# PolusAI/nyxus

Measured on AMD Instinct MI355X. Metric: ROIs/sec (*ALL_GLCM*+*ALL_INTENSITY*, 1024^2 tiles), higher is better.
Workload: dtype f64; 1 GPU; *ALL_GLCM*+*ALL_INTENSITY*, coarse_gray_depth=8, 4 angles, d=1, 1000 synthetic 1024x1024 tiles/GPU x 196 ROIs/tile (disk r=30, 2821 px, bbox 61x61), intensities U[1,4095]; reduce stage on pre-assembled ROI clouds resident in HBM; n_columns=185

## Files before the change

nyxus_amd/csrc/roi_features.hip:

```cpp
#include <hip/hip_runtime.h>
#include <type_traits>
#include <algorithm>
#include <cstdio>
#include "knobs.h"
#include "device_math.h"
#include "roi_kernel.h"
#include "launch_util.h"
#include "glcm_rows.h"
#include "glcm_w64.h"
#include "intensity_close.h"
#include "sort_lds.h"
#include "../../include/nyxhip.h"

namespace nyxhip {


enum { S_MEAN = 0, S_P10, S_P90, S_MEDIAN, S_MODE, S_NG };


template <int NW> __device__ __forceinline__ double xw_chain(const double* s_red, int k)
{
    return NW == 1 ? s_red[k] : ((s_red[k] + s_red[8 + k]) + s_red[16 + k]) + s_red[24 + k];
}
template <int NW> __device__ __forceinline__ double xw_pairs(const double* s_red, int k)
// ... 442 lines not shown
        f[G_DIFAVE] = davg;
        f[G_DIFVAR] = dv;
        f[G_IDMN] = sm[8 + 6];
        f[G_ID] = sm[8 + 7];
        f[G_IDN] = sm[8 + 8];
        f[G_IV] = sm[8 + 9];
        const double r1 = (ent_t - hxy1_t) / hx;
        f[G_INFOMEAS1] = isfinite(r1) ? r1 : soft_nan;
        if (empty)
            for (int k = 0; k < kGlcmAngled; k++) f[k] = soft_nan;
    }
    wav_sync<false>();
}

typedef unsigned short us2_t __attribute__((ext_vector_type(2)));
#ifdef NYX_G16_EXIT
#define G16_EXIT(k, keep) do { if ((k) == NYX_G16_EXIT) { ((double*)blk)[lane & 31] = (double)(keep); return; } } while (0)
#else
#define G16_EXIT(k, keep) do { } while (0)
#endif
template <int NG, int ROLE = 0>
__device__ __forceinline__ void glcm_features_wave64_v2(const uint16_t* P, int Ng_rt, uint32_t* blk, double soft_nan, int lane)
{
    const int Ng = NG ? NG : Ng_rt;
    typedef __attribute__((address_space(3))) const uint16_t lds_cu16_t;
    typedef __attribute__((address_space(3))) const uint32_t lds_cu32_t;
    typedef __attribute__((address_space(3))) uint32_t lds_u32_t;
    const int pitch = (Ng + 3) & ~1;
    double* const f = (double*)blk;
    double* const sm = f + 32;
    double* const T2 = f + 64;
    const bool act = lane < Ng;
    const uint16_t* const Pd = P + pitch;
    G16_EXIT(0, lane);
    uint32_t rc = 0;
    {
        const int nw = (Ng + 1) >> 1;
        lds_cu32_t* rw = (lds_cu32_t*)(uintptr_t)(Pd + (act ? lane : 0) * pitch);
        us2_t a2 = {0, 0};
#pragma unroll 8
        for (int j = 0; j < nw; j++) a2 = a2 + __builtin_bit_cast(us2_t, rw[j]);
        rc = act ? (uint32_t)a2.x + (uint32_t)a2.y : 0u;
    }
    G16_EXIT(1, rc);
    if constexpr (ROLE == 2) {
        const int cj = lane < Ng ? lane : Ng;
        lds_cu16_t* pc = (lds_cu16_t*)(uintptr_t)(Pd + cj);
        uint32_t cc2 = 0;
#pragma unroll 8
        for (int i = 0; i < Ng; i++) cc2 += pc[i * pitch];
        if (!act) cc2 = 0;
        const uint32_t csum2 = wave_sum_t<uint32_t>(rc);
        const double sum_p2 = csum2 == 0 ? 1.0 : (double)csum2;
        const double pcol = fdiv((double)cc2, sum_p2), prow = fdiv((double)rc, sum_p2);
        double hxy1c = 0, hxy2 = 0;
        unsigned long long rem = __ballot(act && rc != 0u);
        while (rem) {
            const int r0 = (int)__builtin_ctzll(rem);
            const uint32_t v = (uint32_t)__builtin_amdgcn_readlane((int)rc, r0);
            const unsigned long long pbits = (unsigned long long)__double_as_longlong(prow);
            const double pr = __longlong_as_double((long long)(((unsigned long long)(uint32_t)__builtin_amdgcn_readlane((int)(uint32_t)(pbits >> 32), r0) << 32) |
                                                               (uint32_t)__builtin_amdgcn_readlane((int)(uint32_t)pbits, r0)));
            unsigned long long grp = __ballot(act && rc == v);
            rem &= ~grp;
            const double pp = pcol * pr;
            const double lg = (double)fast_log2f(pp + 0.000000001);
            hxy2 = __builtin_fma(pp * (double)(uint32_t)__popcll(grp), lg, hxy2);
            uint32_t gsum = 0;
            while (grp) {
                const int r = (int)__builtin_ctzll(grp);
                grp &= grp - 1ull;
                gsum += pc[r * pitch];
            }
            hxy1c = __builtin_fma((double)gsum, lg, hxy1c);
        }
        blk_sync<false>();
        T2[lane] = hxy1c;
        f[lane] = hxy2;
        blk_sync<false>();
        return;
    }
    uint32_t cc = 0, dc = 0;
    uint32_t pxpy_c[2] = {0u, 0u};
    {
        uint32_t W = 0, X = 0;
        const int cj = lane < Ng ? lane : Ng;
        lds_cu16_t* pc = (lds_cu16_t*)(uintptr_t)(Pd + cj);
        lds_u32_t* const b0 = (lds_u32_t*)(uintptr_t)blk;
        lds_u32_t* px = lane == 0 ? b0 : b0 + 128 + lane;
        lds_u32_t* pw = lane == Ng - 1 ? b0 + 64 : b0 + 128 + lane;
#pragma unroll 8
        for (int i = 0; i < Ng; i++) {
            const uint32_t cnt = pc[i * pitch];
            cc += cnt;
            X = lane_plus1_z(X) + cnt;
            W = lane_minus1_z(W) + cnt;
            px[i] = X;
            pw[i] = W;
        }
        wav_sync<false>();
        const uint32_t dlo = act ? blk[lane] : 0u;
        const uint32_t eup = act ? blk[64 + Ng - 1 - lane] : 0u;
        wav_sync<false>();
        const uint32_t wrev = (uint32_t)__builtin_amdgcn_ds_bpermute(4 * (Ng - 1 - lane), (int)W);
        dc = act ? eup + (lane >= 1 ? wrev : 0u) : 0u;
        const int k1 = lane + 64;
        const uint32_t xa = (uint32_t)__builtin_amdgcn_ds_bpermute(4 * (lane - (Ng - 1)), (int)X);
        const uint32_t xb = (uint32_t)__builtin_amdgcn_ds_bpermute(4 * (k1 - (Ng - 1)), (int)X);
        pxpy_c[0] = lane < Ng ? dlo : (lane <= 2 * Ng - 2 ? xa : 0u);
        pxpy_c[1] = k1 <= 2 * Ng - 2 ? xb : 0u;
        if (!act) cc = 0;
    }
    G16_EXIT(2, rc + cc + dc + pxpy_c[0] + pxpy_c[1]);
    const uint32_t csum = wave_sum_t<uint32_t>(rc);
    const bool empty = csum == 0;
    const double sum_p = empty ? 1.0 : (double)csum;
    const double inv_sum_p = fdiv(1.0, sum_p);
    const double pcol = fdiv((double)cc, sum_p), prow = fdiv((double)rc, sum_p), pxmy = fdiv((double)dc, sum_p);
    double pxpy[2] = {0.0, 0.0};
#pragma unroll
    for (int u = 0; u < 2; u++)
        if (lane + 64 * u < 2 * Ng - 1) pxpy[u] = fdiv((double)pxpy_c[u], sum_p);

    {
        const int ca = lane & 7;
        const double pk = (double)ca * inv_sum_p;
        const double t = ca < 7 ? pk * (double)fast_log2f(pk + 0.000000001) : 0.0;
        if (lane < 8) sm[lane] = t;
        wav_sync<false>();
        T2[lane] = t + sm[lane >> 3];
        wav_sync<false>();
    }
    G16_EXIT(3, (uint32_t)(pcol + prow + pxmy + pxpy[0] + pxpy[1]));
    double ent = 0;
    uint32_t asm_i = 0, cmax = 0;
    {
        const int half = (Ng + 1) >> 1, l32 = lane & 31;
        const bool hi = lane >= 32, colp = 2 * l32 < Ng;
        lds_cu32_t* pwd = (lds_cu32_t*)(uintptr_t)(Pd + (hi ? half : 0) * pitch) + (colp ? l32 : 0);
        typedef __attribute__((address_space(3))) const double lds_cd_t;
        lds_cd_t* const T2l = (lds_cd_t*)(uintptr_t)T2;
        us2_t mx = {0, 0};
#pragma unroll 8
        for (int s = 0; s < half; s++) {
            uint32_t w = pwd[s * (pitch >> 1)];
            if (Ng & 1) w = (colp && (!hi || s + half < Ng)) ? w : 0u;
            else if (Ng < 64) w = colp ? w : 0u;
            const us2_t v = __builtin_bit_cast(us2_t, w);
            asm_i = __builtin_amdgcn_udot2(v, v, asm_i, false);
            mx = __builtin_elementwise_max(mx, v);
            const uint32_t m = __builtin_bit_cast(uint32_t, __builtin_elementwise_min(v, (us2_t){7, 7}));
            ent += T2l[(m & 7u) | (m >> 13)];
        }
        cmax = mx.x > mx.y ? (uint32_t)mx.x : (uint32_t)mx.y;
    }
    G16_EXIT(4, (uint32_t)(pcol + prow + pxmy + pxpy[0] + pxpy[1] + ent) + asm_i + cmax);
    double hxy1c = 0, hxy2 = 0;
    if constexpr (ROLE == 0) {
        const int cj = lane < Ng ? lane : Ng;
        lds_cu16_t* pc = (lds_cu16_t*)(uintptr_t)(Pd + cj);
        unsigned long long rem = __ballot(act && rc != 0u);
        while (rem) {
            const int r0 = (int)__builtin_ctzll(rem);
            const uint32_t v = (uint32_t)__builtin_amdgcn_readlane((int)rc, r0);
            const unsigned long long pbits = (unsigned long long)__double_as_longlong(prow);
            const double pr = __longlong_as_double((long long)(((unsigned long long)(uint32_t)__builtin_amdgcn_readlane((int)(uint32_t)(pbits >> 32), r0) << 32) |
                                                               (uint32_t)__builtin_amdgcn_readlane((int)(uint32_t)pbits, r0)));
            unsigned long long grp = __ballot(act && rc == v);
            rem &= ~grp;
            const double pp = pcol * pr;
            const double lg = (double)fast_log2f(pp + 0.000000001);
            hxy2 = __builtin_fma(pp * (double)(uint32_t)__popcll(grp), lg, hxy2);
            uint32_t gsum = 0;
            while (grp) {
                const int r = (int)__builtin_ctzll(grp);
                grp &= grp - 1ull;
                gsum += pc[r * pitch];
            }
            hxy1c = __builtin_fma((double)gsum, lg, hxy1c);
        }
    }
    if (__ballot(cmax >= 7u)) {
        const int cj = lane < Ng ? lane : Ng;
        lds_cu16_t* pc = (lds_cu16_t*)(uintptr_t)(Pd + cj);
        unsigned long long rem = __ballot(act && rc != 0u);
        while (rem) {
            const int r = (int)__builtin_ctzll(rem);
            rem &= rem - 1ull;
            const uint32_t cnt = pc[r * pitch];
            if (cnt >= 7u) { const double p = (double)cnt * inv_sum_p; ent += p * (double)fast_log2f(p + 0.000000001); }
        }
    }
    if constexpr (ROLE == 1) {
        blk_sync<false>();
        blk_sync<false>();
        hxy1c = T2[lane];
        hxy2 = f[lane];
        wav_sync<false>();
    }
    G16_EXIT(5, (uint32_t)(pcol + prow + pxmy + pxpy[0] + pxpy[1] + ent + hxy1c + hxy2) + asm_i + cmax);
    glcm_w64_tail<NG>(Ng, lane, rc, cc, dc, pxpy_c, csum, sum_p, inv_sum_p, pcol, prow, pxmy, pxpy, ent, hxy1c, hxy2, asm_i, cmax, f);
}

#ifdef NYX_STAMP
#define STAMP(i)                                                                          \
    do {                                                                                  \
        unsigned long long t__ = __builtin_readcyclecounter();                            \
        if (tid == 0 && A.stamps) atomicAdd(&A.stamps[i], t__ - t_prev__);                \
        t_prev__ = __builtin_readcyclecounter();                                          \
    } while (0)
#elif defined(NYX_EXIT_AT)
#define STAMP(i) do { if ((i) == NYX_EXIT_AT) return; } while (0)
#else
#define STAMP(i) do { } while (0)
#endif

__constant__ const double kPctFrac[8] = {0.01, 0.1, 0.25, 0.75, 0.9, 0.99, 0.5, 0.5};

typedef __attribute__((address_space(3))) uint8_t lds_u8_t;

typedef const __attribute__((address_space(4))) RoiArgs KArgs;
__device__ __forceinline__ KArgs* late_kernarg()
{
    KArgs* p = (KArgs*)__builtin_amdgcn_kernarg_segment_ptr();
    asm volatile("" : "+s"(p));
    return p;
}
template <bool LATE>
struct KView {
    const RoiArgs& a;
    KArgs* p;
    __device__ __forceinline__ explicit KView(const RoiArgs& a_) : a(a_), p(LATE ? late_kernarg() : nullptr) {}
    __device__ __forceinline__ auto operator->() const
    {
        if constexpr (LATE) return p;
        else return &a;
    }
};
template <bool GS, bool C16, bool SPLIT, bool D8, int FAM = 0, int TIER = 4, bool G16 = false, int WIN = 2, int NW = 4, bool DEFER_P = false>
__device__ __forceinline__ void roi_features_body(const RoiArgs& A, const uint64_t slot)
{
    static_assert((NW == 4 && NW == kMaxAngles) || (NW == 8 && G16 && FAM == 4), "one workgroup of four waves per ROI (and a wave per GLCM angle)");
    constexpr int BS = NW * 64;
    extern __shared__ __attribute__((aligned(16))) unsigned char lds_raw[];
    unsigned char* const lds = GS ? A.sp.scratch + (size_t)blockIdx.x * A.sp.stride : lds_raw;
    const int tid = (int)threadIdx.x, lane = tid & 63, wave = __builtin_amdgcn_readfirstlane(tid >> 6);
    uint64_t roi;
    if (!roi_of_slot(A.sp, slot, A.n_roi, roi))
        return;

    auto reg = [&](uint32_t o) -> unsigned char* { return (GS && o < A.L.gs_lds_bytes) ? lds_raw + o : lds + o; };
    double* s_red = (double*)reg(A.L.red);
    double* s_stat = (double*)reg(A.L.stat);
    uint32_t* s_lbc = (uint32_t*)reg(A.L.lbc);
    uint32_t* s_val = (uint32_t*)(lds + A.L.val);
    using dense_t = typename std::conditional<D8, uint8_t, uint16_t>::type;
    dense_t* s_dense = (dense_t*)(lds + (D8 ? 0u : A.L.dense));
    uint16_t* s_lvlmap = (uint16_t*)reg(A.L.lvlmap);
    uint32_t* s_P = (uint32_t*)reg(A.L.P);
    double* s_g = (double*)reg(A.L.gscr);

    const uint64_t off = A.px_offset[roi];
    const uint32_t n = (uint32_t)(A.px_offset[roi + 1] - off);
    const uint32_t w = A.bbox_w[roi], h = A.bbox_h[roi];
    const uint32_t area = w * h;
    const uint32_t vmin = A.min_inten[roi], vmax = A.max_inten[roi];
    if (!roi_in_launch(A.sp, n, w, h, vmax - vmin))
        return;
    if (vmax - vmin < A.sp.min_range || (A.sp.max_range != 0u && vmax - vmin > A.sp.max_range))
        return;
    constexpr bool FAST = FAM == 1 || FAM == 3;
    constexpr int kRowsTag = 16 + TIER * 4 + (C16 ? 2 : 0) + (D8 ? 1 : 0);
    const bool do_int = FAM == 1 || FAM == 2 || (FAM == 0 && (A.mask & NYXHIP_FAM_INTENSITY) != 0);
    const bool do_glcm = FAM == 1 || FAM == 3 || FAM == 4 || (FAM == 0 && (A.mask & NYXHIP_FAM_GLCM) != 0);
    double* const out_row = A.out + roi * A.ld;
#ifdef NYX_STAMP
    unsigned long long t_prev__ = __builtin_readcyclecounter();
#endif

    const uint32_t range = vmax - vmin;
    const bool use_count = C16 ? do_int : (do_int && A.L.count_cap != 0 && range < A.L.count_cap);
    if (C16 && do_int && range >= A.L.count_cap) {
        if (tid == 0) atomicCAS(A.status, 0, NYXHIP_ERR_ROI_TOO_LARGE);
        return;
    }
    uint32_t* s_cnt = (uint32_t*)reg(A.L.cnt);
    uint32_t P2 = 1;
    while (P2 < n)
        P2 <<= 1;
    const bool radix = !C16 && A.L.radix != 0;
    const bool k16 = radix && A.L.radix_k16 != 0;
    if (n == 0 || (do_int && ((use_count || radix) ? n : P2) > A.L.sort_cap) || (do_glcm && area > A.L.dense_cap)) {
        if (SPLIT && A.glcm_ng && tid == 0)
            A.glcm_ng[roi] = 0;
        if (n != 0 && A.sp.defer_large)
            return;
        if (tid == 0 && n != 0)
            atomicCAS(A.status, 0, NYXHIP_ERR_ROI_TOO_LARGE);
        for (int c = tid; c < A.n_cols; c += BS)
            out_row[c] = __longlong_as_double(0x7ff8000000000000LL);
        return;
    }

    const int greyInfo = A.ibsi ? 0 : A.grey_depth;
    if (FAST) __builtin_assume(greyInfo > 0 && greyInfo <= 16);
    if (G16) __builtin_assume(greyInfo > 16 && greyInfo <= 64);
    const double mslope = greyInfo > 0 ? (double)greyInfo / ((double)vmax - 0.) : 0.0;

    for (int c = tid; c < A.n_cols; c += BS)
        out_row[c] = 0.0;
    if (do_glcm) {
        uint32_t* d32 = (uint32_t*)s_dense;
        for (uint32_t i = tid; i < (D8 ? (area + 64 + 3) / 4 : (area + 1) / 2); i += BS)
            d32[i] = 0;
        if (greyInfo < 0)
            for (uint32_t i = tid; i <= A.L.lvl_cap; i += BS)
                s_lvlmap[i] = 0;
    }
    if (do_int) {
        if (use_count) {
            uint4* c4 = (uint4*)s_cnt;
            const uint32_t n16 = C16 ? (range + 8) / 8 : (range + 4) / 4;
            for (uint32_t i = tid; i < n16; i += BS)
                c4[i] = make_uint4(0, 0, 0, 0);
        } else if (!radix) {
            for (uint32_t i = n + tid; i < P2; i += BS)
                s_val[i] = 0xFFFFFFFFu;
        }
    }
    if (tid < 16)
        s_stat[tid] = 0.0;
    grp_sync<GS, NW>();

    STAMP(0);
    unsigned long long sum = 0, sumsq = 0;
    uint32_t lvl_max = 0;
    constexpr int kU = 4;
    const bool small_v = vmax < (1u << 24);
    const __amdgpu_buffer_rsrc_t rs_v = __builtin_amdgcn_make_buffer_rsrc((void*)(A.inten + off), 0, (int)(n * 4u), 0x00020000);
    const __amdgpu_buffer_rsrc_t rs_x = __builtin_amdgcn_make_buffer_rsrc((void*)(A.x + off), 0, (int)(n * 2u), 0x00020000);
    const __amdgpu_buffer_rsrc_t rs_y = __builtin_amdgcn_make_buffer_rsrc((void*)(A.y + off), 0, (int)(n * 2u), 0x00020000);
    auto trip = [&](auto full_c, auto nz_c, auto tiny_c, uint32_t base) {
        constexpr bool FULL = decltype(full_c)::value, NZ = decltype(nz_c)::value, TINY = decltype(tiny_c)::value;
        uint32_t v[kU], px[kU], py[kU];
#pragma unroll
        for (int u = 0; u < kU; u++) {
            const uint32_t i = base + u * BS + tid;
            v[u] = __builtin_amdgcn_raw_buffer_load_b32(rs_v, (int)(i * 4u), 0, 0);
            px[u] = do_glcm ? (uint32_t)(uint16_t)__builtin_amdgcn_raw_buffer_load_b16(rs_x, (int)(i * 2u), 0, 0) : 0u;
            py[u] = do_glcm ? (uint32_t)(uint16_t)__builtin_amdgcn_raw_buffer_load_b16(rs_y, (int)(i * 2u), 0, 0) : 0u;
        }
        uint32_t s32 = 0, q32 = 0;
        const uint32_t i0 = base + tid;
        uint16_t* const val16 = (uint16_t*)s_val + i0;
#pragma unroll
        for (int u = 0; u < kU; u++) {
            if (!FULL && i0 + u * BS >= n)
                continue;
            if (do_int) {
                if (C16) val16[u * BS] = (uint16_t)(v[u] - vmin);
                else if (k16) ((uint16_t*)s_val)[i0 + u * BS] = (uint16_t)(v[u] - vmin);
                else s_val[i0 + u * BS] = v[u];
                const uint32_t sq = (TINY || small_v) ? (uint32_t)__umul24(v[u], v[u]) : (uint32_t)(v[u] * v[u]);
                if (TINY) { s32 += v[u]; q32 += sq; }
                else { sum += v[u]; sumsq += sq; }
                if (use_count)
                {
                    const uint32_t ci = v[u] - vmin;
                    if (C16) atomicAdd(cnt16_word(s_cnt, ci), 1u << (16 * (ci & 1u)));
                    else atomicAdd(&s_cnt[ci], 1u);
                }
            }
            if (do_glcm) {
                uint32_t lvl = 0;
                if (NZ || v[u] != 0) {
                    if (FAST || G16) {
                        const uint32_t sc = (uint32_t)(mslope * (double)v[u] + 1.0);
                        lvl = sc > (uint32_t)greyInfo ? (uint32_t)greyInfo : sc;
                    } else
                    lvl = greyInfo > 0 ? bin_matlab(v[u], mslope, greyInfo)
                        : greyInfo < 0 ? bin_radiomix(v[u], vmin, vmax, -greyInfo) : v[u];
                    if (greyInfo < 0)
                        s_lvlmap[lvl] = 1;
                    if (greyInfo <= 0)
                        lvl_max = lvl > lvl_max ? lvl : lvl_max;
                }
                const uint32_t cell = __umul24(py[u], w) + px[u];
                if (D8)
                    *(lds_u8_t*)(cell < area ? cell : area + 64) = (uint8_t)lvl;
                else if (cell < area)
                    s_dense[cell] = (dense_t)(lvl > 0xFFFFu ? 0xFFFFu : lvl);
            }
        }
        if (TINY) { sum += s32; sumsq += q32; }
    };
    bool from_window = false;
    if constexpr (WIN != 0 && !GS) {
    if (WIN == 1 || A.win.inten != nullptr) {
        from_window = true;
        const uint32_t L = A.win.label[roi], x0 = A.win.x0[roi];
        const uint64_t tile_px = (uint64_t)A.win.H * A.win.W;
        const bool nz_w = vmin > 0;
        auto member = [&](uint32_t v, uint32_t i, uint32_t cell) {
            if (do_int) {
                if (C16 || k16) ((uint16_t*)s_val)[i] = (uint16_t)(v - vmin);
                else s_val[i] = v;
                sum += v;
                sumsq += small_v ? mul24(v, v) : (uint32_t)(v * v);
                if (use_count) {
                    const uint32_t ci = v - vmin;
                    if (C16) atomicAdd(cnt16_word(s_cnt, ci), 1u << (16 * (ci & 1u)));
                    else atomicAdd(&s_cnt[ci], 1u);
                }
            }
            if (do_glcm) {
                uint32_t lvl = 0;
                if (nz_w || v != 0) {
                    if (FAST || G16) {
                        const uint32_t sc = (uint32_t)(mslope * (double)v + 1.0);
                        lvl = sc > (uint32_t)greyInfo ? (uint32_t)greyInfo : sc;
                    } else
                    lvl = greyInfo > 0 ? bin_matlab(v, mslope, greyInfo) : greyInfo < 0 ? bin_radiomix(v, vmin, vmax, -greyInfo) : v;
                    if (greyInfo < 0) s_lvlmap[lvl] = 1;
                    if (greyInfo <= 0) lvl_max = lvl > lvl_max ? lvl : lvl_max;
                }
                if (D8) *(lds_u8_t*)cell = (uint8_t)lvl;
                else s_dense[cell] = (dense_t)(lvl > 0xFFFFu ? 0xFFFFu : lvl);
            }
        };
        if (w <= 64 && tile_px * 4ull < (1ull << 31)) {
            constexpr int UW = 4;
            const int dtl = A.win.dt_label, dti = A.win.dt_inten;
            auto window_load = [&](auto DTL_c, auto DTI_c) {
            constexpr int DTLc = decltype(DTL_c)::value, DTIc = decltype(DTI_c)::value;
            const int dtl = DTLc ? DTLc : A.win.dt_label, dti = DTIc ? DTIc : A.win.dt_inten;
            const uint32_t Wt = A.win.W;
            const uint64_t tile0 = (uint64_t)A.win.tile[roi] * tile_px;
            const __amdgpu_buffer_rsrc_t rs_l = __builtin_amdgcn_make_buffer_rsrc((void*)((const char*)A.win.lab + tile0 * (uint64_t)dtl), 0, (int)(tile_px * (uint64_t)dtl), 0x00020000);
            const __amdgpu_buffer_rsrc_t rs_i = __builtin_amdgcn_make_buffer_rsrc((void*)((const char*)A.win.inten + tile0 * (uint64_t)dti), 0, (int)(tile_px * (uint64_t)dti), 0x00020000);
            auto ldb = [](const __amdgpu_buffer_rsrc_t& rs, uint32_t voff, uint32_t soff, int dt) -> uint32_t {
                return dt == 4 ? (uint32_t)__builtin_amdgcn_raw_buffer_load_b32(rs, (int)voff, (int)soff, 0)
                     : dt == 2 ? (uint32_t)(uint16_t)__builtin_amdgcn_raw_buffer_load_b16(rs, (int)voff, (int)soff, 0)
                               : (uint32_t)(uint8_t)__builtin_amdgcn_raw_buffer_load_b8(rs, (int)voff, (int)soff, 0);
            };
            const uint32_t e0 = (A.win.y0[roi] + (uint32_t)wave) * Wt + x0;
            const uint32_t vl = (uint32_t)lane * (uint32_t)dtl, vi = (uint32_t)lane * (uint32_t)dti;
            const bool incol = lane < (int)w;
            uint32_t* const s_rc = (uint32_t*)s_red;
            uint32_t base = 0, trip_i = 0;
            for (uint32_t r0 = 0; r0 < h; r0 += NW * UW, trip_i++) {
                uint32_t lb[UW], vv[UW];
                if (incol) {
#pragma unroll
                    for (int u = 0; u < UW; u++)
                        if (r0 + (uint32_t)(u * NW) + (uint32_t)wave < h) {
                            const uint32_t eo = e0 + (r0 + (uint32_t)(u * NW)) * Wt;
                            lb[u] = ldb(rs_l, vl, eo * (uint32_t)dtl, dtl);
                            vv[u] = ldb(rs_i, vi, eo * (uint32_t)dti, dti);
                        }
                }
                unsigned long long bal[UW];
#pragma unroll
                for (int u = 0; u < UW; u++)
                    bal[u] = __ballot(incol && r0 + (uint32_t)(u * NW) + (uint32_t)wave < h && lb[u] == L);
                uint32_t* const rc = s_rc + (trip_i & 1u) * 32u;
                if (lane == 0) {
#pragma unroll
                    for (int u = 0; u < UW; u++) rc[u * NW + wave] = (uint32_t)__popcll(bal[u]);
                }
                grp_sync<GS, NW>();
                const uint32_t inc = wave_scan_u32(lane < NW * UW ? rc[lane & (NW * UW - 1)] : 0u);
#pragma unroll
                for (int u = 0; u < UW; u++) {
                    const uint32_t upto = (uint32_t)__builtin_amdgcn_readlane((int)inc, u * NW + wave);
                    const uint32_t i = base + upto - (uint32_t)__popcll(bal[u])
                                     + __builtin_amdgcn_mbcnt_hi((uint32_t)(bal[u] >> 32), __builtin_amdgcn_mbcnt_lo((uint32_t)bal[u], 0u));
                    if (((bal[u] >> lane) & 1ull) && i < n)
                        member(vv[u], i, (r0 + (uint32_t)(u * NW) + (uint32_t)wave) * w + (uint32_t)lane);
                }
                base += (uint32_t)__builtin_amdgcn_readlane((int)inc, NW * UW - 1);
            }
            grp_sync<GS, NW>();
            };
            using I0 = std::integral_constant<int, 0>; using I1 = std::integral_constant<int, 1>;
            using I2 = std::integral_constant<int, 2>; using I4 = std::integral_constant<int, 4>;
            if (dtl == 4 && dti == 4) window_load(I4{}, I4{});
            else if (dtl == 1 && dti == 2) window_load(I1{}, I2{});
            else if (dtl == 2 && dti == 2) window_load(I2{}, I2{});
            else window_load(I0{}, I0{});
        } else {
        const uint64_t row0 = (uint64_t)A.win.tile[roi] * A.win.H + A.win.y0[roi];
        const uint64_t org = row0 * A.win.W + x0;
        const int dtl = A.win.dt_label, dti = A.win.dt_inten;
        const char* const lab0 = (const char*)A.win.lab + org * (uint64_t)dtl;
        const char* const int0 = (const char*)A.win.inten + org * (uint64_t)dti;
        auto ld = [](const char* p, uint32_t i, int dt) -> uint32_t {
            return dt == 4 ? ((const uint32_t*)p)[i] : dt == 2 ? (uint32_t)((const uint16_t*)p)[i] : (uint32_t)((const uint8_t*)p)[i];
        };
        const uint32_t Wt = A.win.W;
        const uint32_t cw = ((area + BS - 1) / BS) * 64u;
        const uint32_t p_begin = (uint32_t)wave * cw, p_end = p_begin + cw < area ? p_begin + cw : area;
        const uint32_t step_y = 64u / w, step_x = 64u - step_y * w;
        const uint32_t step_o = step_y * Wt + step_x, wrap_o = Wt - w;
        const uint32_t by0 = (p_begin + (uint32_t)lane) / w, bx0 = (p_begin + (uint32_t)lane) - by0 * w;
        const uint32_t off0 = by0 * Wt + bx0;
        uint32_t hits = 0;
        {
            uint32_t bx = bx0, o32 = off0;
            for (uint32_t p = p_begin; p < p_end; p += 64) {
                const bool in = p + (uint32_t)lane < p_end;
                const uint32_t lb = in ? ld(lab0, o32, dtl) : 0u;
                hits += (uint32_t)__popcll(__ballot(in && lb == L));
                bx += step_x; o32 += step_o;
                if (bx >= w) { bx -= w; o32 += wrap_o; }
            }
        }
        uint32_t* const s_hits = (uint32_t*)(s_stat + 12);
        if (lane == 0) s_hits[wave] = hits;
        grp_sync<GS, NW>();
        uint32_t rank0 = 0;
        for (int wv = 0; wv < wave; wv++) rank0 += s_hits[wv];
        const bool nz = vmin > 0;
        uint32_t bx = bx0, by = by0, o32 = off0;
        for (uint32_t p = p_begin; p < p_end; p += 64) {
            const bool in = p + (uint32_t)lane < p_end;
            const uint32_t lb = in ? ld(lab0, o32, dtl) : 0u;
            const uint32_t v = in ? ld(int0, o32, dti) : 0u;
            const bool hit = in && lb == L;
            const unsigned long long bal = __ballot(hit);
            const uint32_t i = rank0 + __builtin_amdgcn_mbcnt_hi((uint32_t)(bal >> 32), __builtin_amdgcn_mbcnt_lo((uint32_t)bal, 0u));
            rank0 += (uint32_t)__popcll(bal);
            if (hit && i < n) {
                if (do_int) {
                    if (C16 || k16) ((uint16_t*)s_val)[i] = (uint16_t)(v - vmin);
                    else s_val[i] = v;
                    sum += v;
                    sumsq += small_v ? (uint32_t)__umul24(v, v) : (uint32_t)(v * v);
                    if (use_count) {
                        const uint32_t ci = v - vmin;
                        if (C16) atomicAdd(cnt16_word(s_cnt, ci), 1u << (16 * (ci & 1u)));
                        else atomicAdd(&s_cnt[ci], 1u);
                    }
                }
                if (do_glcm) {
                    uint32_t lvl = 0;
                    if (nz || v != 0) {
                        if (FAST || G16) {
                            const uint32_t sc = (uint32_t)(mslope * (double)v + 1.0);
                            lvl = sc > (uint32_t)greyInfo ? (uint32_t)greyInfo : sc;
                        } else
                        lvl = greyInfo > 0 ? bin_matlab(v, mslope, greyInfo) : greyInfo < 0 ? bin_radiomix(v, vmin, vmax, -greyInfo) : v;
                        if (greyInfo < 0) s_lvlmap[lvl] = 1;
                        if (greyInfo <= 0) lvl_max = lvl > lvl_max ? lvl : lvl_max;
                    }
                    s_dense[__umul24(by, w) + bx] = D8 ? (dense_t)lvl : (dense_t)(lvl > 0xFFFFu ? 0xFFFFu : lvl);
                }
            }
            bx += step_x; by += step_y; o32 += step_o;
            if (bx >= w) { bx -= w; by++; o32 += wrap_o; }
        }
        }
    }
    }
    if constexpr (WIN != 1) {
    if (!from_window) {
        using T = std::true_type; using F = std::false_type;
        const bool nz = vmin > 0, tiny = vmax < (1u << 15);
        uint32_t base = 0;
        if (nz && tiny) {
            for (; base + kU * BS <= n; base += kU * BS) trip(T{}, T{}, T{}, base);
            if (base < n) trip(F{}, T{}, T{}, base);
        } else {
            for (; base < n; base += kU * BS) trip(F{}, F{}, F{}, base);
        }
    }
    }

    STAMP(1);
    const KView<FAM != 0 || G16> B(A);
    double* const out_row_l = B->out + roi * B->ld;
#ifdef NYX_NO_FUSED
    constexpr bool OVL = false;
#else
    constexpr bool OVL = C16 && !GS && FAM == 1;
#endif
#ifdef NYX_NO_DEFER
    constexpr bool OVL_DEFER = false;
#else
    constexpr bool OVL_DEFER = OVL && DEFER_P;
#endif
    const bool ovl = OVL && B->L.overlap != 0;

    struct FastGlcm {
        int na, Ng, NG1, NN, cells, slot0, slot1, slot2, slot3;
        bool symmetric, usual, dpp2, dpp;
    };
    auto fast_cfg = [&]() -> FastGlcm {
        FastGlcm G;
        G.na = B->glcm_na;
        G.Ng = greyInfo; G.NG1 = G.Ng + 1; G.NN = G.Ng * G.Ng; G.cells = G.NG1 * G.NG1;
        G.symmetric = B->glcm_symmetric != 0;
        G.slot0 = -1; G.slot1 = -1; G.slot2 = -1; G.slot3 = -1;
#pragma unroll
        for (int q = 0; q < kMaxAngles; q++)
            if (q < G.na) {
                const int ang = B->glcm_angles[q];
                if (ang == 0) G.slot0 = q; else if (ang == 45) G.slot1 = q; else if (ang == 90) G.slot2 = q; else G.slot3 = q;
            }
        G.usual = G.slot0 >= 0 && G.slot1 >= 0 && G.slot2 >= 0 && G.slot3 >= 0 && !G.symmetric;
        G.dpp2 = B->glcm_offset == 1 && w > 64 && w <= 128 && G.usual;
        G.dpp = (B->glcm_offset == 1 && w <= 64) || G.dpp2;
        return G;
    };
    auto fast_zero = [&](const FastGlcm& G) {
        for (int i = tid; i < G.na * (G.dpp ? G.cells : G.NN); i += BS)
            s_P[i] = 0;
    };
    auto fast_sweep = [&](const FastGlcm& G, const bool shared) {
        const int na = G.na, Ng = G.Ng, NG1 = G.NG1, NN = G.NN, cells = G.cells;
        const int slot0 = G.slot0, slot1 = G.slot1, slot2 = G.slot2, slot3 = G.slot3;
        const bool symmetric = G.symmetric, usual = G.usual;
        int r_begin, r_end;
        if (shared) {
            r_begin = (int)glcm_row_bounds(h, (uint32_t)wave);
            r_end = (int)glcm_row_bounds(h, (uint32_t)wave + 1u);
        } else {
            r_begin = (int)glcm_row_bounds_even(h, (uint32_t)wave);
            r_end = (int)glcm_row_bounds_even(h, (uint32_t)wave + 1u);
        }
        if (G.dpp2) {
            const uint32_t ng1 = (uint32_t)NG1;
            char* const T0 = (char*)(s_P + slot0 * cells);
            char* const T1 = (char*)(s_P + slot1 * cells);
            char* const T2 = (char*)(s_P + slot2 * cells);
            char* const T3 = (char*)(s_P + slot3 * cells);
            const bool in1 = (uint32_t)lane + 64u < w;
            uint32_t adr0 = (uint32_t)r_begin * w + (uint32_t)lane;
            uint32_t adr1 = in1 ? adr0 + 64u : area + (uint32_t)lane;
            const uint32_t stride1 = in1 ? w : 0u;
            uint32_t c0 = 0, c1 = 0;
            if (r_begin < r_end) { c0 = (uint32_t)(*(const lds_u8_t*)adr0) << 2; c1 = (uint32_t)(*(const lds_u8_t*)adr1) << 2; }
            auto pairs2 = [&](uint32_t c4, uint32_t e, uint32_t se, uint32_t sth, uint32_t sw) {
                if (c4 != 0) {
                    const uint32_t rowb = mul_u24_su(c4, ng1);
                    atomicAdd((uint32_t*)(T0 + rowb + e), 1u);
                    atomicAdd((uint32_t*)(T1 + rowb + se), 1u);
                    atomicAdd((uint32_t*)(T2 + rowb + sth), 1u);
                    atomicAdd((uint32_t*)(T3 + rowb + sw), 1u);
                }
            };
            for (int row = r_begin; row < r_end; row++) {
                adr0 += w; adr1 += stride1;
                const bool below = row + 1 < (int)h;
                const uint32_t n0 = (uint32_t)(*(const lds_u8_t*)adr0) << 2;
                const uint32_t r1 = (uint32_t)(*(const lds_u8_t*)adr1) << 2;
                const uint32_t n1 = below ? r1 : 0u;
                const uint32_t c1_0 = (uint32_t)__builtin_amdgcn_readfirstlane((int)c1), n1_0 = (uint32_t)__builtin_amdgcn_readfirstlane((int)n1);
                const uint32_t n0_63 = readlane63(n0);
                pairs2(c0, lane_plus1(c0, c1_0), lane_plus1(n0, n1_0), n0, lane_minus1_z(n0));
                pairs2(c1, lane_plus1_z(c1), lane_plus1_z(n1), n1, lane_minus1(n1, n0_63));
                c0 = n0; c1 = n1;
            }
        } else
        if (G.dpp) {
            const bool in_col = lane < (int)w;
            const uint32_t ng1 = (uint32_t)NG1;
            char* const T0 = (char*)(s_P + (slot0 >= 0 ? slot0 : 0) * cells);
            char* const T1 = (char*)(s_P + (slot1 >= 0 ? slot1 : 0) * cells);
            char* const T2 = (char*)(s_P + (slot2 >= 0 ? slot2 : 0) * cells);
            char* const T3 = (char*)(s_P + (slot3 >= 0 ? slot3 : 0) * cells);
            uint32_t adr = in_col ? (uint32_t)r_begin * w + (uint32_t)lane : area + (uint32_t)lane - w;
            const uint32_t stride = in_col ? w : 0u;
            uint32_t cur4 = r_begin < r_end ? (uint32_t)(*(const lds_u8_t*)adr) << 2 : 0u;
            adr += stride;
            if (usual) {
                auto pairs = [&](uint32_t c4, uint32_t n4) {
                    const uint32_t nb_e = lane_plus1_z(c4), nb_se = lane_plus1_z(n4), nb_sw = lane_minus1_z(n4);
                    if (c4 != 0) {
                        const uint32_t rowb = mul_u24_su(c4, ng1);
                        atomicAdd((uint32_t*)(T0 + rowb + nb_e), 1u);
                        atomicAdd((uint32_t*)(T1 + rowb + nb_se), 1u);
                        atomicAdd((uint32_t*)(T2 + rowb + n4), 1u);
                        atomicAdd((uint32_t*)(T3 + rowb + nb_sw), 1u);
                    }
                };
                int row = r_begin;
                for (; row + 1 < r_end; row += 2) {
                    const uint32_t n4a = (uint32_t)(*(const lds_u8_t*)adr) << 2;
                    pairs(cur4, n4a);
                    const uint32_t n4b = (uint32_t)(*(const lds_u8_t*)(adr + stride)) << 2;
                    pairs(n4a, n4b);
                    cur4 = n4b;
                    adr += 2 * stride;
                }
                if (row < r_end)
                    pairs(cur4, (uint32_t)(*(const lds_u8_t*)adr) << 2);
            } else {
                const int has0 = slot0 >= 0, has1 = slot1 >= 0, has2 = slot2 >= 0, has3 = slot3 >= 0;
                for (int row = r_begin; row < r_end; row++, adr += stride) {
                    const uint32_t nxt4 = (uint32_t)(*(const lds_u8_t*)adr) << 2;
                    const uint32_t nb_e = lane_plus1_z(cur4), nb_se = lane_plus1_z(nxt4), nb_sw = lane_minus1_z(nxt4);
                    if (cur4 != 0) {
                        const uint32_t rowb = mul_u24_su(cur4, ng1);
                        if (has0) atomicAdd((uint32_t*)(T0 + rowb + nb_e), 1u);
                        if (has1) atomicAdd((uint32_t*)(T1 + rowb + nb_se), 1u);
                        if (has2) atomicAdd((uint32_t*)(T2 + rowb + nxt4), 1u);
                        if (has3) atomicAdd((uint32_t*)(T3 + rowb + nb_sw), 1u);
                        if (symmetric) {
                            if (has0) atomicAdd((uint32_t*)(T0 + mul_u24_su(nb_e, ng1) + cur4), 1u);
                            if (has1) atomicAdd((uint32_t*)(T1 + mul_u24_su(nb_se, ng1) + cur4), 1u);
                            if (has2) atomicAdd((uint32_t*)(T2 + mul_u24_su(nxt4, ng1) + cur4), 1u);
                            if (has3) atomicAdd((uint32_t*)(T3 + mul_u24_su(nb_sw, ng1) + cur4), 1u);
                        }
                    }
                    cur4 = nxt4;
                }
            }
        } else {
            for (int row = wave; row < (int)h; row += NW)
                for (int col = lane; col < (int)w; col += 64) {
                    const uint32_t lb = s_dense[(uint32_t)row * w + (uint32_t)col];
                    if (lb == 0)
                        continue;
#pragma unroll
                    for (int q = 0; q < kMaxAngles; q++) {
                        if (q >= na)
                            break;
                        const int ang = B->glcm_angles[q];
                        const int dx = ang == 90 ? 0 : ang == 135 ? -B->glcm_offset : B->glcm_offset, dy = ang == 0 ? 0 : B->glcm_offset;
                        const int r2 = row + dy, c2 = col + dx;
                        if (r2 < 0 || r2 >= (int)h || c2 < 0 || c2 >= (int)w)
                            continue;
                        const uint32_t la = s_dense[(uint32_t)r2 * w + (uint32_t)c2];
                        if (la == 0)
                            continue;
                        atomicAdd(&s_P[q * NN + ((int)lb - 1) * Ng + (int)la - 1], 1u);
                        if (symmetric)
                            atomicAdd(&s_P[q * NN + ((int)la - 1) * Ng + (int)lb - 1], 1u);
                    }
                }
        }
    };
    if (do_int) {
        double* o = out_row_l + B->col_intensity;
        const double dn = (double)n;
        if ((unsigned long long)n * vmax < (1ull << 32))
            sum = wave_sum_t<uint32_t>((uint32_t)sum);
        else
            sum = wave_sum_u64(sum);
        if (C16) {
            const uint32_t lo24 = wave_sum_t<uint32_t>((uint32_t)sumsq & 0xFFFFFFu), hi = wave_sum_t<uint32_t>((uint32_t)(sumsq >> 24));
            sumsq = ((unsigned long long)hi << 24) + lo24;
        } else
            sumsq = wave_sum_u64(sumsq);
        if (lane == 0) {
            s_red[wave * 8 + 0] = (double)sum;
            s_red[wave * 8 + 1] = (double)sumsq;
        }
        grp_sync<GS, NW>();
        const bool blank = (vmin == 0 && vmax == 0);
#if defined(NYX_NO_FUSED) || defined(NYX_NO_DEFER)
        constexpr bool DEFER = false;
#else
        constexpr bool DEFER = DEFER_P && C16 && !GS;
#endif
        const bool defer = DEFER && !blank;
        double* const rec = DEFER ? B->close_rec + roi * kCloseRec : nullptr;
        if (tid == 0) {
            double tot = 0, totsq = 0;
            for (int wv = 0; wv < NW; wv++) {
                tot += s_red[wv * 8 + 0];
                totsq += s_red[wv * 8 + 1];
            }
            const double mean = tot / dn;
            s_stat[S_MEAN] = mean;
            if (FAST)
                s_stat[S_NG] = bin_pixel(vmin, vmin, vmax, B->glcm_grey_depth) == bin_pixel(vmax, vmin, vmax, B->glcm_grey_depth) ? 1.0 : 0.0;
            if (defer) {
                rec[CR_TOT] = tot;
                rec[CR_TOTSQ] = totsq;
            } else {
                close_sums(RowColumns{o}, dn, vmin, vmax, tot, totsq, mean, B->slide_min && B->slide_max,
                           [&] { return B->slide_max[roi] - B->slide_min[roi]; }, blank);
            }
        }
        grp_sync<GS, NW>();
        const double mean = s_stat[S_MEAN];
        STAMP(2);

        const double binW100 = (double)range / 100.;
        const uint32_t nb = (uint32_t)B->n_hist;
        auto idx100 = [=](uint32_t v) -> int {
            double realIdx = (double)(v - vmin) / binW100;
            return (realIdx != realIdx) ? 0 : (int)realIdx;
        };

        const uint32_t Q = ((range + 1 + NW * 512 - 1) / (NW * 512)) * 512;
        uint32_t* const s_woff = (uint32_t*)(s_stat + 8);
#ifdef NYX_NO_FUSED
        constexpr bool FUSED = false;
#else
        constexpr bool FUSED = C16 && !GS;
#endif
        uint32_t* const s_fm = (uint32_t*)(lds + B->L.fm);
        uint32_t* const s_foff = (uint32_t*)(s_stat + 12);
        auto eng_put = [&](int k, uint32_t v) {
            if (OVL) ((uint32_t*)(s_red + wave * 8 + 6))[k] = v;
            else s_red[wave * 8 + k] = (double)v;
        };
        auto eng_get = [&](int wv, int k) -> uint32_t {
            return OVL ? ((const uint32_t*)(s_red + wv * 8 + 6))[k] : (uint32_t)s_red[wv * 8 + k];
        };
        double acc[6] = {0, 0, 0, 0, 0, 0};
        auto central_sweep = [&]() {
            const double meanx = mean - (double)vmin;
            auto px1 = [&](uint32_t x) {
                const double d = (double)x - meanx;
                const double d2 = d * d;
                acc[0] += fabs(d);
                acc[1] = __builtin_fma(d, d, acc[1]);
                acc[2] = __builtin_fma(d2, d, acc[2]);
                acc[3] = __builtin_fma(d2, d2, acc[3]);
                const double d4 = d2 * d2;
                acc[4] = __builtin_fma(d4, d, acc[4]);
                acc[5] = __builtin_fma(d4, d2, acc[5]);
            };
            const uint16_t* const pv = (const uint16_t*)s_val + tid;
            const uint32_t n_full = (uint32_t)__builtin_amdgcn_readfirstlane((int)(n / BS)), n_rem = n - n_full * BS;
            {
                uint32_t k = 0;
                for (; k + 1 < n_full; k += 2) { px1(pv[k * BS]); px1(pv[(k + 1) * BS]); }
                if (k < n_full) px1(pv[k * BS]);
            }
            if ((uint32_t)tid < n_rem)
                px1(pv[n_full * BS]);
            {
                double t[8];
#pragma unroll
                for (int k = 0; k < 8; k++) t[k] = k < 6 ? acc[k] : 0.0;
                const double tot = wave_transpose_sum8(t, lane);
                if ((lane & 7) == 0 && (lane >> 3) < 6)
                    s_red[wave * 8 + (lane >> 3)] = tot;
            }
            grp_sync<GS, NW>();
            if (DEFER) {
                if (tid < 6)
                    rec[CR_ACC + tid] = xw_chain<NW>(s_red, tid);
                if (!OVL && tid == 0)
                    B->close_flag[roi] = 1u;
            } else {
                if (tid == 0) {
                    double a6[6];
#pragma unroll
                    for (int k = 0; k < 6; k++) {
                        a6[k] = xw_chain<NW>(s_red, k);
                        asm volatile("" : "+v"(a6[k]) :: "memory");
                    }
                    close_central<CovDiv::ieee>(RowColumns{o}, a6, n, dn, mean, blank);
                }
                if (!OVL)
                    grp_sync<GS, NW>();
            }
        };
        if (OVL) {
            if (!blank)
                central_sweep();
            if (ovl)
                fast_zero(fast_cfg());
        }
        if (use_count) {
            uint32_t carry = 0, best_c = 0, best_i = 0;
// ... 1376 lines not shown
```

Before: 107.3 million ROIs/s.

## Software-pipeline ROI cloud loads and hoist first batch above LDS init

Adds a rotated loader for the compact builds. It issues the next trip's buffer loads (intensity, x, y) right after each element of the current trip is consumed, so global-memory latency overlaps the LDS scatter and binning work. It also issues the first batch of loads before the LDS zeroing and group barrier, hiding the initial load latency behind setup. Scheduling barriers and empty asm constraints pin the instruction order. The cost is more live registers, which may lower occupancy, and extra template variants.

```diff
diff --git a/nyxus_amd/csrc/roi_features.hip b/nyxus_amd/csrc/roi_features.hip
--- a/nyxus_amd/csrc/roi_features.hip
+++ b/nyxus_amd/csrc/roi_features.hip
@@ -768,6 +768,47 @@
         return;
     }
 
+    constexpr int kU = 4;
+#ifdef NYX_NO_TRIP_ROTATE
+    constexpr bool ROTATE = false;
+#else
+    constexpr bool ROTATE = (FAM == 1 || FAM == 2 || FAM == 3) && !GS && !G16 && WIN != 1;
+#endif
+#if defined(NYX_NO_TRIP_HOIST) || (defined(NYX_EXIT_AT) && NYX_EXIT_AT <= 0)
+    constexpr bool HOIST = false;
+#else
+    constexpr bool HOIST = ROTATE;
+#endif
+    struct Trip { uint32_t v[kU], px[kU], py[kU]; };
+    struct Trip16 { uint32_t v[kU]; uint16_t px[kU], py[kU]; };
+    struct Cloud { __amdgpu_buffer_rsrc_t v, x, y; };
+    [[maybe_unused]] Trip rot{};
+    [[maybe_unused]] Trip16 first{};
+    [[maybe_unused]] Cloud cl;
+    [[maybe_unused]] auto issue_to = [&](auto& t, int u, uint32_t base) {
+        const uint32_t i = base + u * BS + tid;
+        t.v[u] = __builtin_amdgcn_raw_buffer_load_b32(cl.v, (int)(i * 4u), 0, 0);
+        if (do_glcm) {
+            t.px[u] = (uint16_t)__builtin_amdgcn_raw_buffer_load_b16(cl.x, (int)(i * 2u), 0, 0);
+            t.py[u] = (uint16_t)__builtin_amdgcn_raw_buffer_load_b16(cl.y, (int)(i * 2u), 0, 0);
+        }
+        __builtin_amdgcn_sched_barrier(0);
+    };
+    [[maybe_unused]] auto issue = [&](int u, uint32_t base) { issue_to(rot, u, base); };
+    if constexpr (ROTATE) {
+        cl.v = __builtin_amdgcn_make_buffer_rsrc((void*)(A.inten + off), 0, (int)(n * 4u), 0x00020000);
+        cl.x = __builtin_amdgcn_make_buffer_rsrc((void*)(A.x + off), 0, (int)(n * 2u), 0x00020000);
+        cl.y = __builtin_amdgcn_make_buffer_rsrc((void*)(A.y + off), 0, (int)(n * 2u), 0x00020000);
+    }
+    if constexpr (HOIST) {
+        bool cloud = true;
+        if constexpr (WIN != 0) cloud = A.win.inten == nullptr;
+        if (cloud) {
+#pragma unroll
+            for (int u = 0; u < kU; u++) issue_to(first, u, 0u);
+        }
+    }
+
     const int greyInfo = A.ibsi ? 0 : A.grey_depth;
     if (FAST) __builtin_assume(greyInfo > 0 && greyInfo <= 16);
     if (G16) __builtin_assume(greyInfo > 16 && greyInfo <= 64);
@@ -797,11 +838,11 @@
     if (tid < 16)
         s_stat[tid] = 0.0;
     grp_sync<GS, NW>();
+    if constexpr (HOIST) __builtin_amdgcn_sched_barrier(0);
 
     STAMP(0);
     unsigned long long sum = 0, sumsq = 0;
     uint32_t lvl_max = 0;
-    constexpr int kU = 4;
     const bool small_v = vmax < (1u << 24);
     const __amdgpu_buffer_rsrc_t rs_v = __builtin_amdgcn_make_buffer_rsrc((void*)(A.inten + off), 0, (int)(n * 4u), 0x00020000);
     const __amdgpu_buffer_rsrc_t rs_x = __builtin_amdgcn_make_buffer_rsrc((void*)(A.x + off), 0, (int)(n * 2u), 0x00020000);
@@ -859,6 +900,45 @@
             }
         }
         if (TINY) { sum += s32; sumsq += q32; }
+    };
+    [[maybe_unused]] auto consume = [&](auto full_c, auto nz_c, auto tiny_c, int u, uint32_t base, uint32_t& s32, uint32_t& q32) {
+        if constexpr (ROTATE) {
+            static_assert(C16 && D8 && (FAM == 2 || FAST), "the rotated loader serves the compact builds only");
+            constexpr bool FULL = decltype(full_c)::value, NZ = decltype(nz_c)::value, TINY = decltype(tiny_c)::value;
+            const uint32_t i = base + u * BS + tid, val = rot.v[u];
+            if (!FULL && i >= n)
+                return;
+            if (do_int) {
+                ((uint16_t*)s_val)[i] = (uint16_t)(val - vmin);
+                const uint32_t sq = (TINY || small_v) ? (uint32_t)__umul24(val, val) : (uint32_t)(val * val);
+                if (TINY) { s32 += val; q32 += sq; }
+                else { sum += val; sumsq += sq; }
+                const uint32_t ci = val - vmin;
+                atomicAdd(cnt16_word(s_cnt, ci), 1u << (16 * (ci & 1u)));
+            }
+            if (do_glcm) {
+                uint32_t lvl = 0;
+                if (NZ || val != 0) {
+                    const uint32_t sc = (uint32_t)(mslope * (double)val + 1.0);
+                    lvl = sc > (uint32_t)greyInfo ? (uint32_t)greyInfo : sc;
+                }
+                const uint32_t cell = __umul24(rot.py[u], w) + rot.px[u];
+                *(lds_u8_t*)(cell < area ? cell : area + 64) = (uint8_t)lvl;
+            }
+        }
+    };
+    [[maybe_unused]] auto trip_rot = [&](auto full_c, auto nz_c, auto tiny_c, auto next_c, uint32_t base) {
+        uint32_t s32 = 0, q32 = 0;
+#pragma unroll
+        for (int u = 0; u < kU; u++) {
+            consume(full_c, nz_c, tiny_c, u, base, s32, q32);
+            if (!do_int) { }
+            else if (decltype(tiny_c)::value) asm volatile("" : "+v"(s32), "+v"(q32));
+            else asm volatile("" : "+v"(sum), "+v"(sumsq));
+            __builtin_amdgcn_sched_barrier(0);
+            if (decltype(next_c)::value) issue(u, base + kU * BS);
+        }
+        if (decltype(tiny_c)::value) { sum += s32; sumsq += q32; }
     };
     bool from_window = false;
     if constexpr (WIN != 0 && !GS) {
@@ -1033,6 +1113,28 @@
         using T = std::true_type; using F = std::false_type;
         const bool nz = vmin > 0, tiny = vmax < (1u << 15);
         uint32_t base = 0;
+        if constexpr (ROTATE) {
+            auto widen = [&] {
+                if constexpr (HOIST) {
+#pragma unroll
+                    for (int u = 0; u < kU; u++) { rot.v[u] = first.v[u]; rot.px[u] = first.px[u]; rot.py[u] = first.py[u]; }
+                } else {
+#pragma unroll
+                    for (int u = 0; u < kU; u++) issue(u, 0u);
+                }
+            };
+            if (nz && tiny) {
+                widen();
+                for (; base + kU * BS <= n; base += kU * BS) trip_rot(T{}, T{}, T{}, T{}, base);
+                if (base < n) trip_rot(F{}, T{}, T{}, F{}, base);
+            } else {
+                widen();
+                for (; base + kU * BS < n; base += kU * BS) trip_rot(T{}, F{}, F{}, T{}, base);
+                trip_rot(F{}, F{}, F{}, F{}, base);
+                constexpr int kWaitVmcnt0 = 0x0F70;
+                __builtin_amdgcn_s_waitcnt(kWaitVmcnt0);
+            }
+        } else
         if (nz && tiny) {
             for (; base + kU * BS <= n; base += kU * BS) trip(T{}, T{}, T{}, base);
             if (base < n) trip(F{}, T{}, T{}, base);
```

New measurement: 111.0 million ROIs/s (median of 6 runs). 1.03x the previous value.
